# Prachet-Dev-Singh/DenseCLIP_Vit_multimodal

Hardware: AMD Instinct MI355X
Metric: images/sec (fwd+bwd) ViT-B/16 DenseCLIP @1024x2048 (higher is better)
Workload: dtype bf16

## Files before the change

denseclip_vit_multimodal_amd/csrc/attention_bwd1.hip:

```cpp
#include "dkdv_frag.h"

namespace {

constexpr int B1_NW = 4, B1_KB = 64 * B1_NW;
typedef Dkv2Ctx<bf16, B1_NW> B1Ring;
constexpr int B1_RING = 4 * B1Ring::SLOT;
constexpr int B1_W0 = B1_RING;
constexpr int B1_SMEM = B1_W0 + B1_KB * 4;
constexpr int B1_IMG = B1_KB * 128;
static_assert(B1_SMEM + 2 * B1_IMG <= 160 * 1024, "LDS");

__device__ __forceinline__ int lane_now() {
    int l;
    asm volatile("v_mbcnt_lo_u32_b32 %0, -1, 0\n\tv_mbcnt_hi_u32_b32 %0, -1, %0" : "=v"(l));
    return l;
}

template <typename F>
__device__ __forceinline__ F to_agpr(F v) {
    F r;
    asm volatile("" : "=a"(r) : "0"(v));
    return r;
}

// ... 92 lines not shown
    seeds(S0, P0, nb, nsub, h);
    fence();
}

template <typename T>
__device__ __forceinline__ void dq_tile(f32x16& acc, const char* kimg, const char* dsimg, int qb, int db) {
    typedef typename Mfma<T>::frag frag;
    const int lane = threadIdx.x & 63;
    const DsTrBase dsb = ds_tr_base(qb, lane);
    frag a[2], b[2];
    a[0] = tr_frag<T>(kimg, 0, 0, db, lane);
    b[0] = trds_frag<T>(dsimg, dsb, 0, 0);
    acc = zero16();
#pragma unroll
    for (int ks = 0; ks < 16; ++ks) {
        if (ks + 1 < 16) {
            a[(ks + 1) & 1] = tr_frag<T>(kimg, (ks + 1) >> 1, (ks + 1) & 1, db, lane);
            b[(ks + 1) & 1] = trds_frag<T>(dsimg, dsb, (ks + 1) >> 1, (ks + 1) & 1);
        }
        acc = Mfma<T>::mma(a[ks & 1], b[ks & 1], acc);
    }
}

template <typename T>
__device__ __forceinline__ void store_dq_half(rsrc_t rp, uint32_t rs, uint32_t row0, int db, const f32x16& acc,
                                              float scale) {
    typedef T t2 __attribute__((ext_vector_type(2)));
    unsigned w[4][2];
#pragma unroll
    for (int g = 0; g < 4; ++g)
#pragma unroll
        for (int j = 0; j < 2; ++j) {
            const float a0 = acc[4 * g + 2 * j], a1 = acc[4 * g + 2 * j + 1];
            const t2 p = std::is_same<T, bf16>::value ? t2{(T)a0, (T)a1} : t2{(T)(a0 * scale), (T)(a1 * scale)};
            w[g][j] = __builtin_bit_cast(unsigned, p);
        }
    const int lane = lane_now();
    const uint32_t vo = (uint32_t)(lane & 31) * rs + (uint32_t)(16 * (lane >> 5) + 64 * db);
    const uint32_t so = row0 * rs;
    typedef unsigned u32x4 __attribute__((ext_vector_type(4)));
#pragma unroll
    for (int G = 0; G < 4; G += 2) {
#pragma unroll
        for (int j = 0; j < 2; ++j) {
            const auto r = __builtin_amdgcn_permlane32_swap(w[G][j], w[G + 1][j], false, false);
            w[G][j] = r[0];
            w[G + 1][j] = r[1];
        }
        const u32x4 v = {w[G][0], w[G][1], w[G + 1][0], w[G + 1][1]};
        __builtin_amdgcn_raw_buffer_store_b128(v, rp, vo + 16 * G, so, 0);
    }
}

struct B1Out {
    rsrc_t part;
    uint32_t rs;
    int qb, db;
    float sc;
};

template <typename T, int Q>
__device__ __forceinline__ void step1(Dkv2Ctx<T, 4>& c, K6<T>& k, int t, typename Mfma<T>::frag (&qa)[4],
                                      typename Mfma<T>::frag (&ga)[4], f32x16& S0, f32x16& P0, f32x16& dq,
                                      const B1Out& out, char* kimg, char* dsimg) {
    typedef Dkv2Ctx<T, 4> X;
    wait_vmcnt<X::PIECES + 1>();
    __builtin_amdgcn_s_barrier();
    asm volatile("" ::: "memory");
    if (t > 0)
        store_dq_half<T>(out.part, out.rs, (uint32_t)(64 * (t - 1) + 1 + out.qb * 32), out.db, dq, out.sc);
    dkv2_issue<T, 4>(c, t + 3 < c.nt ? t + 3 : c.nt - 1, (Q + 3) & 3);
    const char* cur = c.smem + Q * X::SLOT;
    const char* nxt = c.smem + ((Q + 1) & 3) * X::SLOT;
    sub1<T, 0>(k, c.h, c.l32, c.lane, cur, cur, 1, qa, ga, S0, P0, dsimg, c.wave);
    sub1<T, 1>(k, c.h, c.l32, c.lane, cur, nxt, 0, qa, ga, S0, P0, dsimg, c.wave);
    asm volatile("s_waitcnt lgkmcnt(0)" ::: "memory");
    __builtin_amdgcn_s_barrier();
    asm volatile("" ::: "memory");
    fence();
    dq_tile<T>(dq, kimg, dsimg, out.qb, out.db);
    fence();
}

template <typename T>
__global__ __launch_bounds__(256, 1) void attn_bwd1_kernel(const T* __restrict__ qkv, const T* __restrict__ dout,
                                                           const float* __restrict__ lse,
                                                           const float* __restrict__ delta,
                                                           const float* __restrict__ nlse,
                                                           const float* __restrict__ ndelta, T* __restrict__ dqkv,
                                                           T* __restrict__ dqpart, int N, int H, float dk_scale,
                                                           float scale, float* __restrict__ r0q) {
    constexpr int NW = B1_NW, KB = B1_KB;
    typedef Dkv2Ctx<T, NW> X;
    typedef typename Mfma<T>::frag frag;
    static_assert(X::SLOT == B1Ring::SLOT, "ring geometry");
    __shared__ __attribute__((aligned(128))) char smem[B1_SMEM];
    __shared__ __attribute__((aligned(128))) char kimg[B1_IMG];
    __shared__ __attribute__((aligned(128))) char dsimg[B1_IMG];
    X c;
    K6<T> k;
    c.smem = smem;
    c.lane = threadIdx.x & 63;
    c.wave = __builtin_amdgcn_readfirstlane(threadIdx.x >> 6);
    c.h = c.lane >> 5;
    c.l32 = c.lane & 31;
    const int nkb = (N - 1 + KB - 1) / KB;
    const int tile = xcd_remap(blockIdx.x, gridDim.x);
    const int kblk = tile % nkb, bh = tile / nkb, b = bh / H, hd = bh % H;
    const int C = H * HD;
    const int64_t ld = 3 * (int64_t)C;
    const T* Bb = qkv + (int64_t)b * N * ld;
// ... 312 lines not shown
        fence();
        asm volatile("" : "+a"(k.vf[1][s]));
        P1 = Mfma<T>::mma(ga[s], k.vf[1][s], P1);
        fin_chunk<T>(S0, P0, k0, 2 * s + 1);
        fence();
    }
    dq_mma2<T, 8 * SUB + 2, false>(dq, kt, dbf);
    fence();
    dq_load2<T, 8 * SUB + 4>(dbf, dsprev, dqo);
#pragma unroll
    for (int s = 0; s < 2; ++s) {
        mfma_acc<T, false>(k.dv[0][0], gt[s][0], as_frag<T>(k0.p[s]));
        fin_chunk<T>(S1, P1, k1, 4 * s);
        fence();
        mfma_acc<T, false>(k.dv[0][1], gt[s][1], as_frag<T>(k0.p[s]));
        fin_chunk<T>(S1, P1, k1, 4 * s + 1);
        fence();
        mfma_acc<T, false>(k.dk[0][0], qt[s][0], as_frag<T>(k0.d[s]));
        fin_chunk<T>(S1, P1, k1, 4 * s + 2);
        fence();
        mfma_acc<T, false>(k.dk[0][1], qt[s][1], as_frag<T>(k0.d[s]));
        fin_chunk<T>(S1, P1, k1, 4 * s + 3);
        fence();
    }
    load_qg_x<T>(qa, ga, nb, nsub, l32, h);
    dq_mma2<T, 8 * SUB + 4, false>(dq, kt, dbf);
    fence();
    dq_load2<T, 8 * SUB + 6>(dbf, dsprev, dqo);
    const uint32_t dsw = ds_put_base(wave, lane);
    ds_put<SUB, 0>(dscur, dsw, k0.d);
#pragma unroll
    for (int s = 0; s < 2; ++s) {
        mfma_acc<T, true>(k.dv[1][0], gt[s][0], as_frag<T>(k1.p[s]));
        mfma_acc<T, false>(k.dv[1][1], gt[s][1], as_frag<T>(k1.p[s]));
        mfma_acc<T, false>(k.dk[1][0], qt[s][0], as_frag<T>(k1.d[s]));
        mfma_acc<T, false>(k.dk[1][1], qt[s][1], as_frag<T>(k1.d[s]));
    }
    ds_put<SUB, 1>(dscur, dsw, k1.d);
    seeds(S0, P0, nb, nsub, h);
    dq_mma2<T, 8 * SUB + 6, false>(dq, kt, dbf);
    fence();
}

template <typename T, int Q, int DB>
__device__ __forceinline__ void step2(Dkv2Ctx<T, 4>& c, K6<T>& k, int t, typename Mfma<T>::frag (&qa)[4],
                                      typename Mfma<T>::frag (&ga)[4], f32x16& S0, f32x16& P0, f32x16& dq,
                                      const B1Out& out, const DqOps& dqo, const typename Mfma<T>::frag (&kt)[16],
                                      char* dsimg) {
    typedef Dkv2Ctx<T, 4> X;
    wait_vmcnt<X::PIECES + 1>();
    asm volatile("s_waitcnt lgkmcnt(0)" ::: "memory");
    __builtin_amdgcn_s_barrier();
    asm volatile("" ::: "memory");
    dkv2_issue<T, 4>(c, t + 3 < c.nt ? t + 3 : c.nt - 1, (Q + 3) & 3);
    const char* cur = c.smem + Q * X::SLOT;
    const char* nxt = c.smem + ((Q + 1) & 3) * X::SLOT;
    char* dscur = dsimg + DB * B1_IMG;
    const char* dsprev = dsimg + (DB ^ 1) * B1_IMG;
    sub2<T, 0>(k, c.h, c.l32, c.lane, c.wave, cur, cur, 1, qa, ga, S0, P0, dq, kt, dscur, dsprev, dqo, &out,
               t >= 2 ? (uint32_t)(64 * (t - 2) + 1 + out.qb * 32) : 0xFFFFFFFFu);
    sub2<T, 1>(k, c.h, c.l32, c.lane, c.wave, cur, nxt, 0, qa, ga, S0, P0, dq, kt, dscur, dsprev, dqo);
}

template <typename T>
__device__ __forceinline__ void dq_tile_kt(f32x16& acc, const typename Mfma<T>::frag (&kt)[16], const char* dsimg,
                                           const DqOps& dqo) {
    typename Mfma<T>::frag b[2];
    dq_load2<T, 0>(b, dsimg, dqo);
    dq_mma2<T, 0, true>(acc, kt, b);
#pragma unroll
    for (int ks = 2; ks < 16; ks += 2) {
        switch (ks) {
            case 2: dq_load2<T, 2>(b, dsimg, dqo); dq_mma2<T, 2, false>(acc, kt, b); break;
            case 4: dq_load2<T, 4>(b, dsimg, dqo); dq_mma2<T, 4, false>(acc, kt, b); break;
            case 6: dq_load2<T, 6>(b, dsimg, dqo); dq_mma2<T, 6, false>(acc, kt, b); break;
            case 8: dq_load2<T, 8>(b, dsimg, dqo); dq_mma2<T, 8, false>(acc, kt, b); break;
            case 10: dq_load2<T, 10>(b, dsimg, dqo); dq_mma2<T, 10, false>(acc, kt, b); break;
            case 12: dq_load2<T, 12>(b, dsimg, dqo); dq_mma2<T, 12, false>(acc, kt, b); break;
            default: dq_load2<T, 14>(b, dsimg, dqo); dq_mma2<T, 14, false>(acc, kt, b); break;
        }
    }
}

template <typename T>
struct B1pArgs {
    const T *qkv, *dout;
    const float *lse, *delta, *nlse, *ndelta;
    T *dqkv, *dqpart;
    int N, H;
    float dk_scale, scale;
    float* r0q;
    int tiles, nbh;
    int period;
    unsigned* state;
    const float* ds0v;
};

template <typename T, bool P>
__device__ __forceinline__ int bwd1b_tile(const T* __restrict__ qkv, const T* __restrict__ dout,
                                          const float* __restrict__ lse, const float* __restrict__ delta,
                                          const float* __restrict__ nlse, const float* __restrict__ ndelta,
                                          T* __restrict__ dqkv, T* __restrict__ dqpart, int N, int H, float dk_scale,
                                          float scale, float* __restrict__ r0q, int tile, int pend, int wave,
                                          __attribute__((address_space(4))) const B1pArgs<T>* ka) {
    constexpr int NW = B1_NW, KB = B1_KB;
    typedef Dkv2Ctx<T, NW> X;
    typedef typename Mfma<T>::frag frag;
    static_assert(X::SLOT == B1Ring::SLOT, "ring geometry");
    __shared__ __attribute__((aligned(128))) char smem[B2_SMEM];
    __shared__ __attribute__((aligned(128))) char dsimg[2 * B1_IMG];
    char* kimg = dsimg + B1_IMG;
    X c;
    K6<T> k;
    c.smem = smem;
    c.lane = P ? lane_now() : (int)(threadIdx.x & 63);
    c.wave = P ? wave : __builtin_amdgcn_readfirstlane(threadIdx.x >> 6);
    if constexpr (P) asm volatile("" : "+s"(N), "+s"(H), "+s"(c.wave));
    c.h = c.lane >> 5;
    c.l32 = c.lane & 31;
    const int nkb = (N - 1 + KB - 1) / KB;
    const int kblk = tile % nkb, bh = tile / nkb, b = bh / H, hd = bh % H;
    const int C = H * HD;
    const int64_t ld = 3 * (int64_t)C;
    const T* Bb = qkv + (int64_t)b * N * ld;
    const T* dOb = dout + (int64_t)b * N * C;
    c.ldq = (uint32_t)(ld * sizeof(T));
    c.ldg = (uint32_t)(C * sizeof(T));
    c.nt = (N - 1 + 63) / 64;
    c.rem = N - 1 - 64 * (c.nt - 1);
    B1Out out;
    out.rs = (uint32_t)nkb * 128;
    out.part = make_rsrc((const char*)dqpart + ((size_t)bh * (size_t)(1 + 64 * c.nt) * nkb + kblk) * 128,
                         (uint32_t)(1 + 64 * c.nt) * out.rs);
    out.qb = c.wave >> 1;
    out.db = c.wave & 1;
    out.sc = scale / DsScale<T>::v;
    DqOps dqo;
    dqo.db = out.db;
    dqo.dsb = ds_tr_base(out.qb, c.lane);
    int key[2];
    bool kok[2];
#pragma unroll
    for (int kb = 0; kb < 2; ++kb) {
        key[kb] = 1 + kblk * KB + c.wave * 64 + kb * 32 + c.l32;
        kok[kb] = key[kb] < N;
        const int kc = kok[kb] ? key[kb] : N - 1;
#pragma unroll
        for (int s = 0; s < 4; ++s) {
            k.kf[kb][s] = *(const frag*)(Bb + (int64_t)kc * ld + C + hd * HD + (2 * s + c.h) * 8);
            k.vf[kb][s] = *(const frag*)(Bb + (int64_t)kc * ld + 2 * C + hd * HD + (2 * s + c.h) * 8);
        }
    }
    frag q0[4], g0[4];
#pragma unroll
    for (int s = 0; s < 4; ++s) {
        q0[s] = *(const frag*)(Bb + hd * HD + (2 * s + c.h) * 8);
        g0[s] = *(const frag*)(dOb + hd * HD + (2 * s + c.h) * 8);
    }
    typedef T t4 __attribute__((ext_vector_type(4)));
    t4 q0d[2][4], g0d[2][4];
#pragma unroll
    for (int db = 0; db < 2; ++db)
#pragma unroll
        for (int g = 0; g < 4; ++g) {
            q0d[db][g] = *(const t4*)(Bb + hd * HD + db * 32 + 8 * g + 4 * c.h);
            g0d[db][g] = *(const t4*)(dOb + hd * HD + db * 32 + 8 * g + 4 * c.h);
        }
    const float L0 = lse[(int64_t)bh * N], d0 = delta[(int64_t)bh * N];

    c.rs = make_rsrc(Bb, (uint32_t)N * c.ldq);
    c.rg = make_rsrc(dOb, (uint32_t)N * c.ldg);
    c.rl = make_rsrc(nlse + (int64_t)bh * N, (uint32_t)N * 4);
    c.rd = make_rsrc(ndelta + (int64_t)bh * N, (uint32_t)N * 4);
    const bool q_wave = c.wave * X::PIECES < 8;
    c.rmine = q_wave ? c.rs : c.rg;
    c.ldmine = q_wave ? c.ldq : c.ldg;
#pragma unroll
    for (int i = 0; i < X::PIECES; ++i) {
        const int piece = c.wave * X::PIECES + i;
        const int r = (piece & 7) * 8 + (c.lane >> 3);
        const uint32_t chunk = (uint32_t)(((c.lane & 7) ^ xsw(r)) * 16);
        c.voff[i] = piece < 8 ? (uint32_t)r * c.ldq + chunk + (uint32_t)(hd * HD * sizeof(T))
                              : (uint32_t)r * c.ldg + chunk + (uint32_t)(hd * HD * sizeof(T));
    }
    dkv2_issue<T, NW>(c, 0, 0);
    dkv2_issue<T, NW>(c, c.nt > 1 ? 1 : 0, 1);
    dkv2_issue<T, NW>(c, c.nt > 2 ? 2 : c.nt - 1, 2);

#pragma unroll
    for (int kb = 0; kb < 2; ++kb) {
        const int row = c.wave * 64 + kb * 32 + c.l32;
#pragma unroll
        for (int s = 0; s < 4; ++s) {
            frag v = k.kf[kb][s];
            if (!kok[kb])
#pragma unroll
                for (int j = 0; j < 8; ++j) v[j] = (T)0.f;
            *(frag*)(kimg + row * 128 + (((2 * s + c.h) ^ xsw(row)) << 4)) = v;
        }
    }
#pragma unroll
    for (int kb = 0; kb < 2; ++kb) {
        float spart = 0.f, ppart = 0.f;
#pragma unroll
        for (int s = 0; s < 4; ++s)
#pragma unroll
            for (int j = 0; j < 8; ++j) {
                spart += (float)q0[s][j] * (float)k.kf[kb][s][j];
                ppart += (float)g0[s][j] * (float)k.vf[kb][s][j];
            }
        const float p0 = __builtin_amdgcn_exp2f(xhalf_sum(spart) - L0);
        const float ds0 = p0 * (xhalf_sum(ppart) - d0) * DsScale<T>::v;
        ((float*)(smem + B2_RING))[c.wave * 64 + kb * 32 + c.l32] = kok[kb] ? ds0 : 0.f;
#pragma unroll
        for (int db = 0; db < 2; ++db)
#pragma unroll
            for (int g = 0; g < 4; ++g)
#pragma unroll
                for (int e = 0; e < 4; ++e) {
                    k.dv[kb][db][4 * g + e] = p0 * (float)g0d[db][g][e];
                    k.dk[kb][db][4 * g + e] = ds0 * (float)q0d[db][g][e];
                }
#pragma unroll
        for (int s = 0; s < 4; ++s) frag_ds_scale<T>(k.vf[kb][s]);
    }

    wait_vmcnt<2 * (X::PIECES + 1)>();
    asm volatile("s_waitcnt lgkmcnt(0)" ::: "memory");
    __builtin_amdgcn_s_barrier();
    asm volatile("" ::: "memory");
    frag qa[4], ga[4], kt[16];
    f32x16 S0, P0, dq;
#pragma unroll
    for (int ks = 0; ks < 16; ++ks) kt[ks] = to_agpr(tr_frag<T>(kimg, ks >> 1, ks & 1, dqo.db, c.lane));
    load_qg<T>(qa, ga, smem, 0, c.l32, c.h);
    seeds(S0, P0, smem, 0, c.h);
    int t = 0;
    for (; t + 4 <= c.nt; t += 4) {
        step2<T, 0, 0>(c, k, t, qa, ga, S0, P0, dq, out, dqo, kt, dsimg);
        step2<T, 1, 1>(c, k, t + 1, qa, ga, S0, P0, dq, out, dqo, kt, dsimg);
        step2<T, 2, 0>(c, k, t + 2, qa, ga, S0, P0, dq, out, dqo, kt, dsimg);
        step2<T, 3, 1>(c, k, t + 3, qa, ga, S0, P0, dq, out, dqo, kt, dsimg);
    }
    if (t < c.nt) step2<T, 0, 0>(c, k, t++, qa, ga, S0, P0, dq, out, dqo, kt, dsimg);
    if (t < c.nt) step2<T, 1, 1>(c, k, t++, qa, ga, S0, P0, dq, out, dqo, kt, dsimg);
    if (t < c.nt) step2<T, 2, 0>(c, k, t++, qa, ga, S0, P0, dq, out, dqo, kt, dsimg);
    wait_vmcnt<0>();
    asm volatile("s_waitcnt lgkmcnt(0)" ::: "memory");
    __builtin_amdgcn_s_barrier();
    asm volatile("" ::: "memory");
    if (c.nt >= 2) {
        dq_settle(dq);
        store_dq_half<T>(out.part, out.rs, (uint32_t)(64 * (c.nt - 2) + 1 + out.qb * 32), out.db, dq, out.sc);
    }
    dq_tile_kt<T>(dq, kt, dsimg + ((c.nt - 1) & 1) * B1_IMG, dqo);
    dq_settle(dq);
    store_dq_half<T>(out.part, out.rs, (uint32_t)(64 * (c.nt - 1) + 1 + out.qb * 32), out.db, dq, out.sc);
    wait_vmcnt<0>();
    unsigned duty = 0;
    if (r0q != nullptr) {
        __syncthreads();
        const int lane = P ? lane_now() : (int)__lane_id();
        float* part = (float*)(smem + NW * 64 * 128);
        gu32* state = nullptr;
        if constexpr (P) {
            asm volatile("" : "+s"(ka));
            state = (gu32*)ka->state;
            if (c.wave == NW - 1 && lane == 0) {
                __builtin_amdgcn_fence(__ATOMIC_RELEASE, "agent");
                asm volatile("s_waitcnt vmcnt(0)" ::: "memory");
                __hip_atomic_fetch_add(state + bh, 1u, __ATOMIC_RELAXED, __HIP_MEMORY_SCOPE_AGENT);
                unsigned ready = 0;
                for (int j = 0; j < pend; ++j) {
                    const int u = tile - (j + 1) * (int)gridDim.x;
                    if (u >= 0 && __hip_atomic_load(state + u / nkb, __ATOMIC_RELAXED, __HIP_MEMORY_SCOPE_AGENT) ==
                                      (unsigned)nkb)
                        ready |= 1u << j;
                }
                ((unsigned*)part)[NW * 64] = ready;
            }
        }
        char* img = smem + c.wave * 64 * 128;
        r0_put<T>(img, k.kf[0], lane & 31, lane >> 5);
        r0_put<T>(img, k.kf[1], 32 + (lane & 31), lane >> 5);
        const float aq = r0_colsum<T, 64>(img, (const float*)(smem + B2_RING) + c.wave * 64, lane);
        part[c.wave * 64 + lane] = aq;
        __syncthreads();
        if constexpr (P) {
            duty = __builtin_amdgcn_readfirstlane(((const unsigned*)part)[NW * 64]);
            if (duty && c.wave == NW - 1 && lane == 0) {
                __builtin_amdgcn_fence(__ATOMIC_ACQUIRE, "agent");
                asm volatile("s_waitcnt vmcnt(0)" ::: "memory");
            }
        }
        if (c.wave == 0) {
            float sum = 0.f;
#pragma unroll
            for (int v = 0; v < NW; ++v) sum += part[v * 64 + lane];
            r0q[((int64_t)bh * nkb + kblk) * 64 + lane] = sum;
        }
    }
    asm volatile("s_nop 7\n\ts_nop 7\n\ts_nop 3"
                 : "+a"(k.dk[0][0]), "+a"(k.dk[0][1]), "+a"(k.dk[1][0]), "+a"(k.dk[1][1]), "+a"(k.dv[0][0]),
                   "+a"(k.dv[0][1]), "+a"(k.dv[1][0]), "+a"(k.dv[1][1]));
#pragma unroll
    for (int kb = 0; kb < 2; ++kb) {
        if (kok[kb]) {
            T* rk = dqkv + ((int64_t)b * N + key[kb]) * ld + C + hd * HD;
            store_row_t21<T>(rk, k.dk[kb], dk_scale / DsScale<T>::v, c.h);
            store_row_t21<T>(rk + C, k.dv[kb], 1.0f, c.h);
        }
    }
    if constexpr (P) {
        if (duty) {
            __syncthreads();
            asm volatile("" : "+s"(ka));
            const T* pp = ka->dqpart;
            const int nrb = (N - 1 + 31) / 32, per = (nrb + nkb - 1) / nkb;
            const int tid = c.wave * 64 + lane_now();
            for (int j = 0; j < pend; ++j) {
                if (!(duty >> j & 1)) continue;
                const int u = tile - j * (int)gridDim.x, pbh = (u - (int)gridDim.x) / nkb, share = u % nkb;
                const int rb1 = min((share + 1) * per, nrb);
                for (int rb = share * per; rb < rb1; rb += DUTY_R) {
                    const int nr = min(DUTY_R, rb1 - rb);
                    dq_reduce_rows<T, DUTY_R>(pp, ka->ds0v, ka->qkv, ka->dqkv, N, H, nkb, pbh, rb, nr,
                                              ka->scale / DsScale<T>::v, tid);
                    if (tid < nr)
                        __hip_atomic_store((gu32*)ka->state + bwd1b_reduced_at(ka->nbh, pbh, nrb, rb + tid), 1u,
                                           __ATOMIC_RELAXED, __HIP_MEMORY_SCOPE_AGENT);
                }
            }
        }
        __syncthreads();
    }
    return bh;
}

template <typename T>
__global__ __launch_bounds__(256, 1) void attn_bwd1b_kernel(const T* __restrict__ qkv, const T* __restrict__ dout,
                                                            const float* __restrict__ lse,
                                                            const float* __restrict__ delta,
                                                            const float* __restrict__ nlse,
                                                            const float* __restrict__ ndelta, T* __restrict__ dqkv,
                                                            T* __restrict__ dqpart, int N, int H, float dk_scale,
                                                            float scale, float* __restrict__ r0q) {
    bwd1b_tile<T, false>(qkv, dout, lse, delta, nlse, ndelta, dqkv, dqpart, N, H, dk_scale, scale, r0q,
                         xcd_remap(blockIdx.x, gridDim.x), 0, 0, nullptr);
}

template <typename T>
__global__ __launch_bounds__(256, 1) void attn_bwd1p_kernel(const B1pArgs<T> args) {
    typedef __attribute__((address_space(4))) const B1pArgs<T> kargs_t;
    const int wave = __builtin_amdgcn_readfirstlane(threadIdx.x >> 6);
    const int period = args.period;
    int owed = 0, round = blockIdx.x / 8;
    for (int tile = xcd_remap(blockIdx.x, gridDim.x); tile < args.tiles; tile += gridDim.x, ++round) {
        kargs_t* ka = (kargs_t*)__builtin_amdgcn_kernarg_segment_ptr();
        asm volatile("" : "+s"(ka));
        ++owed;
        const bool now = period > 0 && (round % period == period - 1 || tile + (int)gridDim.x >= ka->tiles);
        bwd1b_tile<T, true>(ka->qkv, ka->dout, ka->lse, ka->delta, ka->nlse, ka->ndelta, ka->dqkv, ka->dqpart, ka->N,
                            ka->H, ka->dk_scale, ka->scale, ka->r0q, tile, now ? owed : 0, wave, ka);
        if (now || period <= 0) owed = 0;
    }
}

template <typename T>
__global__ __launch_bounds__(256) void attn_bwd1_prep_kernel(const T* __restrict__ qkv, const T* __restrict__ o,
                                                             const T* __restrict__ dout, const float* __restrict__ lse,
                                                             float* __restrict__ delta, float* __restrict__ nstat,
                                                             float* __restrict__ ds0v, float* __restrict__ r0kv, int N,
                                                             int H, int nqp, int head_minor) {
    typedef typename Mfma<T>::frag frag;
    constexpr int QB = 128;
    __shared__ __attribute__((aligned(16))) char smem[4 * 32 * 128 + 2 * QB * 4 + 4 * 128 * 4];
    const int lane = threadIdx.x & 63, wave = threadIdx.x >> 6, h = lane >> 5, l32 = lane & 31;
    int blk, bh;
    if (head_minor) {
        const int hm = blockIdx.x % H, r = blockIdx.x / H;
        blk = r % nqp;
        bh = (r / nqp) * H + hm;
    } else {
        blk = blockIdx.x % nqp;
        bh = blockIdx.x / nqp;
    }
    const int b = bh / H, hd = bh % H;
    const int C = H * HD;
    const int64_t ld = 3 * (int64_t)C;
    const T* Bb = qkv + (int64_t)b * N * ld;
    const T* dOb = dout + (int64_t)b * N * C + hd * HD;
    const int q = 1 + blk * QB + wave * 32 + l32;
    const bool qok = q < N;
    const int qc = qok ? q : N - 1;
    frag qf[4], gf[4], of[4], k0[4], v0[4];
    const T* Orow = o + ((int64_t)b * N + qc) * C + hd * HD;
#pragma unroll
    for (int s = 0; s < 4; ++s) {
        k0[s] = *(const frag*)(Bb + C + hd * HD + (2 * s + h) * 8);
        v0[s] = *(const frag*)(Bb + 2 * C + hd * HD + (2 * s + h) * 8);
        qf[s] = *(const frag*)(Bb + (int64_t)qc * ld + hd * HD + (2 * s + h) * 8);
        gf[s] = *(const frag*)(dOb + (int64_t)qc * C + (2 * s + h) * 8);
        of[s] = *(const frag*)(Orow + (2 * s + h) * 8);
    }
    const float L = lse[(int64_t)bh * N + qc];
    float dpart = 0.f, spart = 0.f, ppart = 0.f;
#pragma unroll
    for (int s = 0; s < 4; ++s)
#pragma unroll
        for (int j = 0; j < 8; ++j) {
            dpart += (float)of[s][j] * (float)gf[s][j];
            spart += (float)qf[s][j] * (float)k0[s][j];
            ppart += (float)gf[s][j] * (float)v0[s][j];
        }
    const float dl = xhalf_sum(dpart);
    const float p0 = __builtin_amdgcn_exp2f(xhalf_sum(spart) - L);
// ... 42 lines not shown
    if (state != nullptr && __hip_atomic_load((const gu32*)state + bwd1b_reduced_at(gridDim.x / nrb, bh, nrb, rb),
                                              __ATOMIC_RELAXED, __HIP_MEMORY_SCOPE_AGENT) != 0)
        return;
    dq_reduce_rows<T, 1>(dqpart, ds0v, qkv, dqkv, N, H, nkb, bh, rb, 1, sc, threadIdx.x);
}

constexpr int RQ_Q = 8;
constexpr int RQ_MAX_NKB = 56;
template <typename T>
__global__ __launch_bounds__(256) void attn_bwd1_dq_reduce_lds(const T* __restrict__ dqpart,
                                                               const float* __restrict__ ds0v,
                                                               const T* __restrict__ qkv, T* __restrict__ dqkv,
                                                               int N, int H, int nkb, int nrb, float sc,
                                                               const unsigned* state) {
    typedef T t2 __attribute__((ext_vector_type(2)));
    typedef unsigned u32x4 __attribute__((ext_vector_type(4)));
    extern __shared__ __attribute__((aligned(16))) char rq_lds[];
    const int rb = blockIdx.x % nrb, bh = blockIdx.x / nrb, b = bh / H, hd = bh % H;
    if (state != nullptr &&
        __hip_atomic_load((const gu32*)state + bwd1b_reduced_at(gridDim.x / nrb, bh, (N - 1 + 31) / 32, rb / (32 / RQ_Q)),
                          __ATOMIC_RELAXED, __HIP_MEMORY_SCOPE_AGENT) != 0)
        return;
    const int q0 = 1 + rb * RQ_Q;
    const int C = H * HD;
    const int64_t ld = 3 * (int64_t)C;
    const int64_t Np = 1 + 64 * (int64_t)((N - 1 + 63) / 64);
    const int run = nkb * 128, stride = run + 128;
    const char* src = (const char*)(dqpart + ((int64_t)bh * Np + q0) * nkb * 64);
    const int chunks = RQ_Q * nkb * 8;
    for (int c = threadIdx.x; c < chunks; c += 256) {
        const int qi = c / (nkb * 8), w = c - qi * (nkb * 8);
        const u32x4 v = __builtin_nontemporal_load((const u32x4*)(src + (int64_t)c * 16));
        *(u32x4*)(rq_lds + qi * stride + w * 16) = v;
    }
    __syncthreads();
    const int qi = threadIdx.x >> 5, cp = threadIdx.x & 31;
    const int q = q0 + qi;
    if (q >= N) return;
    const t2 kv = *(const t2*)(qkv + (int64_t)b * N * ld + C + hd * HD + 2 * cp);
    constexpr bool unscaled = std::is_same<T, bf16>::value;
    const float w = ds0v[(int64_t)bh * N + q] * (unscaled ? 1.0f : sc);
    float a0 = w * (float)kv[0], a1 = w * (float)kv[1];
    const char* row = rq_lds + qi * stride + cp * 4;
#pragma unroll 8
    for (int j = 0; j < nkb; ++j) {
        const t2 v = *(const t2*)(row + j * 128);
        a0 += (float)v[0];
        a1 += (float)v[1];
    }
    const t2 r = {(T)(unscaled ? a0 * sc : a0), (T)(unscaled ? a1 * sc : a1)};
    *(t2*)(dqkv + ((int64_t)b * N + q) * ld + hd * HD + 2 * cp) = r;
}

int bwd1_cu_count() {
    int dev = 0, c = 0;
    if (hipGetDevice(&dev) != hipSuccess ||
        hipDeviceGetAttribute(&c, hipDeviceAttributeMultiprocessorCount, dev) != hipSuccess || c <= 0)
        c = 256;
    return c;
}

template <typename T>
void bwd1_launch(const void* qkv, const void* o, const void* dout, const float* lse, float* delta, float* nstat,
                 float* ds0v, float* r0kv, int nqp, float* r0q, void* dqpart, void* dqkv, int B, int N, int H,
                 float scale, unsigned* state, hipStream_t st) {
    const int nkb = (N - 1 + B1_KB - 1) / B1_KB, tiles = B * H * nkb;
    attn_bwd1_prep_kernel<T><<<B * H * nqp, 256, 0, st>>>((const T*)qkv, (const T*)o, (const T*)dout, lse, delta, nstat,
                                                          ds0v, r0kv, N, H, nqp,
                                                          dclip_option(DCLIP_OPT_ATTN_PREP_ORDER) == 1);
    const int blk = dclip_option(DCLIP_OPT_ATTN_BWD_BLOCK), cap = dclip_option(DCLIP_OPT_ATTN_BWD_WGS);
    const int G = cap > 0 ? cap : bwd1_cu_count();
    const bool persistent = blk == 0 && state != nullptr && r0q != nullptr && tiles > G;
    if (!persistent) state = nullptr;
    if (persistent) {
        (void)hipMemsetAsync(state, 0, (size_t)attn_bwd1_state_bytes(B, N, H), st);
        const B1pArgs<T> args = {(const T*)qkv, (const T*)dout, lse,   delta,  nstat, nstat + (int64_t)B * H * N,
                                 (T*)dqkv,      (T*)dqpart,     N,     H,      1.0f / LOG2E, scale,
                                 r0q,           tiles,          B * H, DUTY_PERIOD, state, ds0v};
        attn_bwd1p_kernel<T><<<G, 256, 0, st>>>(args);
    } else if (blk != 9)
        attn_bwd1b_kernel<T><<<B * H * nkb, 256, 0, st>>>((const T*)qkv, (const T*)dout, lse, delta, nstat,
                                                          nstat + (int64_t)B * H * N, (T*)dqkv, (T*)dqpart, N, H,
                                                          1.0f / LOG2E, scale, r0q);
    else
        attn_bwd1_kernel<T><<<B * H * nkb, 256, 0, st>>>((const T*)qkv, (const T*)dout, lse, delta, nstat,
                                                         nstat + (int64_t)B * H * N, (T*)dqkv, (T*)dqpart, N, H,
                                                         1.0f / LOG2E, scale, r0q);
    if (dclip_option(DCLIP_OPT_ATTN_DQ_REDUCE) == 1 && nkb <= RQ_MAX_NKB) {
        const int nrb = (N - 1 + RQ_Q - 1) / RQ_Q;
        attn_bwd1_dq_reduce_lds<T><<<B * H * nrb, 256, RQ_Q * (nkb * 128 + 128), st>>>(
            (const T*)dqpart, ds0v, (const T*)qkv, (T*)dqkv, N, H, nkb, nrb, scale / DsScale<T>::v, state);
        return;
    }
    const int nrb = (N - 1 + 31) / 32;
    attn_bwd1_dq_reduce<T><<<B * H * nrb, 256, 0, st>>>((const T*)dqpart, ds0v, (const T*)qkv, (T*)dqkv, N, H, nkb, nrb,
                                                        scale / DsScale<T>::v, state);
}

}

int attn_bwd1_prep_blocks(int N) { return (N - 1 + 127) / 128; }

int64_t attn_bwd1_part_bytes(int B, int N, int H) {
    const int64_t nkb = (N - 1 + B1_KB - 1) / B1_KB, np = 1 + 64 * (int64_t)((N - 1 + 63) / 64);
    return (int64_t)B * H * nkb * np * 128;
}

int64_t attn_bwd1_state_bytes(int B, int N, int H) {
    const int64_t words = (int64_t)B * H * (1 + (N - 1 + 31) / 32);
    return (words * 4 + 255) / 256 * 256;
}

void attn_bwd1_launch(int dt, const void* qkv, const void* o, const void* dout, const float* lse, float* delta,
                      float* nstat, float* ds0v, float* r0kv, float* r0q, void* dqpart, void* dqkv, int B, int N,
                      int H, float scale, hipStream_t st, void* state) {
    const int nqp = attn_bwd1_prep_blocks(N);
    if (dt == DCLIP_BF16)
        bwd1_launch<bf16>(qkv, o, dout, lse, delta, nstat, ds0v, r0kv, nqp, r0q, dqpart, dqkv, B, N, H, scale,
                          (unsigned*)state, st);
    else
        bwd1_launch<f16>(qkv, o, dout, lse, delta, nstat, ds0v, r0kv, nqp, r0q, dqpart, dqkv, B, N, H, scale,
                         (unsigned*)state, st);
}
```

Measured before the change: 64.88.

## Prefetch next persistent tile's K/V/CLS rows into LDS across the tile seam

In the persistent attention backward kernel, the next tile's K/V rows, the CLS q/dout rows and its first three ring stages are issued as async buffer-to-LDS loads while the current tile finishes its dq tail, r0 fold and dK/dV stores. At the start of the next tile the fragments are read from LDS instead of global memory. The goal is to hide global-load latency at the boundary between tiles. The r0 fold is moved earlier into a dedicated LDS region, __syncthreads calls are replaced with raw barriers, and hipMemsetAsync is replaced with a small zeroing kernel. It also adds optional timestamp diagnostics. This costs extra LDS and adds staging-buffer aliasing hazards.

```diff
diff --git a/denseclip_vit_multimodal_amd/csrc/attention_bwd1.hip b/denseclip_vit_multimodal_amd/csrc/attention_bwd1.hip
--- a/denseclip_vit_multimodal_amd/csrc/attention_bwd1.hip
+++ b/denseclip_vit_multimodal_amd/csrc/attention_bwd1.hip
@@ -168,11 +168,43 @@
     }
 }
 
+#ifndef DCLIP_BWD1_SEAM_PREFETCH
+#define DCLIP_BWD1_SEAM_PREFETCH 1
+#endif
+enum {
+    B1_PT_RT0 = 0,
+    B1_PT_TOP = 1,
+    B1_PT_LOOP = 2,
+    B1_PT_LEFT = 3,
+    B1_PT_DQ = 4,
+    B1_PT_PUB = 5,
+    B1_PT_DKDV = 6,
+    B1_PT_END = 7,
+    B1_PT_RT1 = 8,
+    B1_PTS = 16
+};
+#ifdef DCLIP_BWD1_SEAM_DIAG
+constexpr int B1_DIAG_TILES = 4096;
+__device__ unsigned long long g_seam_stamps[B1_DIAG_TILES * B1_PTS];
+#define B1_STAMP_V(tile, pt, who, val)                                                              \
+    do {                                                                                            \
+        if ((who) && (tile) >= 0 && (tile) < B1_DIAG_TILES) g_seam_stamps[(tile) * B1_PTS + (pt)] = (val); \
+    } while (0)
+#define B1_STAMP(tile, pt, who) B1_STAMP_V(tile, pt, who, __builtin_amdgcn_s_memtime())
+#define B1_STAMP_RT(tile, pt, who) B1_STAMP_V(tile, pt, who, __builtin_amdgcn_s_memrealtime())
+#else
+#define B1_STAMP(tile, pt, who) do { } while (0)
+#define B1_STAMP_RT(tile, pt, who) do { } while (0)
+#endif
+
 struct B1Out {
     rsrc_t part;
     uint32_t rs;
     int qb, db;
     float sc;
+#ifdef DCLIP_BWD1_SEAM_DIAG
+    int diag_tile;
+#endif
 };
 
 template <typename T, int Q>
@@ -591,6 +623,9 @@
     asm volatile("s_waitcnt lgkmcnt(0)" ::: "memory");
     __builtin_amdgcn_s_barrier();
     asm volatile("" ::: "memory");
+#ifdef DCLIP_BWD1_SEAM_DIAG
+    if constexpr (Q == 0) B1_STAMP(out.diag_tile, B1_PT_LOOP, t == 0 && c.wave == 0 && lane_now() == 0);
+#endif
     dkv2_issue<T, 4>(c, t + 3 < c.nt ? t + 3 : c.nt - 1, (Q + 3) & 3);
     const char* cur = c.smem + Q * X::SLOT;
     const char* nxt = c.smem + ((Q + 1) & 3) * X::SLOT;
@@ -635,30 +670,30 @@
     const float* ds0v;
 };
 
-template <typename T, bool P>
-__device__ __forceinline__ int bwd1b_tile(const T* __restrict__ qkv, const T* __restrict__ dout,
-                                          const float* __restrict__ lse, const float* __restrict__ delta,
-                                          const float* __restrict__ nlse, const float* __restrict__ ndelta,
-                                          T* __restrict__ dqkv, T* __restrict__ dqpart, int N, int H, float dk_scale,
-                                          float scale, float* __restrict__ r0q, int tile, int pend, int wave,
-                                          __attribute__((address_space(4))) const B1pArgs<T>* ka) {
-    constexpr int NW = B1_NW, KB = B1_KB;
-    typedef Dkv2Ctx<T, NW> X;
-    typedef typename Mfma<T>::frag frag;
-    static_assert(X::SLOT == B1Ring::SLOT, "ring geometry");
-    __shared__ __attribute__((aligned(128))) char smem[B2_SMEM];
-    __shared__ __attribute__((aligned(128))) char dsimg[2 * B1_IMG];
-    char* kimg = dsimg + B1_IMG;
-    X c;
-    K6<T> k;
-    c.smem = smem;
-    c.lane = P ? lane_now() : (int)(threadIdx.x & 63);
-    c.wave = P ? wave : __builtin_amdgcn_readfirstlane(threadIdx.x >> 6);
-    if constexpr (P) asm volatile("" : "+s"(N), "+s"(H), "+s"(c.wave));
+constexpr int B1_CLS = B2_RING;
+constexpr int B1_FOLD_W0 = 0, B1_FOLD_PART = B1_KB * 4, B1_FOLD_READY = B1_FOLD_PART + B1_NW * 64 * 4;
+constexpr int B1_FOLD = B1_FOLD_READY + 128;
+constexpr int B1_VST = (B1_NW - 1) * 64 * 128;
+static_assert(B2_SMEM + 2 * B1_IMG + B1_FOLD + B1_VST <= 160 * 1024, "LDS");
+static_assert(64 * 128 <= B1Ring::SLOT, "wave 3's V stage in ring slot 3");
+
+template <typename T>
+struct B1Pre {
+    typename Mfma<T>::frag kf[2][4], vf[2][4];
+    typename Mfma<T>::frag q0[4], g0[4];
+    typedef T t4 __attribute__((ext_vector_type(4)));
+    t4 q0d[2][4], g0d[2][4];
+};
+
+template <typename T>
+__device__ __forceinline__ void b1_ring_ctx(Dkv2Ctx<T, B1_NW>& c, const T* __restrict__ qkv,
+                                            const T* __restrict__ dout, const float* __restrict__ nlse,
+                                            const float* __restrict__ ndelta, int N, int H, int tile) {
+    typedef Dkv2Ctx<T, B1_NW> X;
     c.h = c.lane >> 5;
     c.l32 = c.lane & 31;
-    const int nkb = (N - 1 + KB - 1) / KB;
-    const int kblk = tile % nkb, bh = tile / nkb, b = bh / H, hd = bh % H;
+    const int nkb = (N - 1 + B1_KB - 1) / B1_KB;
+    const int bh = tile / nkb, b = bh / H, hd = bh % H;
     const int C = H * HD;
     const int64_t ld = 3 * (int64_t)C;
     const T* Bb = qkv + (int64_t)b * N * ld;
@@ -667,6 +702,157 @@
     c.ldg = (uint32_t)(C * sizeof(T));
     c.nt = (N - 1 + 63) / 64;
     c.rem = N - 1 - 64 * (c.nt - 1);
+    c.rs = make_rsrc(Bb, (uint32_t)N * c.ldq);
+    c.rg = make_rsrc(dOb, (uint32_t)N * c.ldg);
+    c.rl = make_rsrc(nlse + (int64_t)bh * N, (uint32_t)N * 4);
+    c.rd = make_rsrc(ndelta + (int64_t)bh * N, (uint32_t)N * 4);
+    const bool q_wave = c.wave * X::PIECES < 8;
+    c.rmine = q_wave ? c.rs : c.rg;
+    c.ldmine = q_wave ? c.ldq : c.ldg;
+#pragma unroll
+    for (int i = 0; i < X::PIECES; ++i) {
+        const int piece = c.wave * X::PIECES + i;
+        const int r = (piece & 7) * 8 + (c.lane >> 3);
+        const uint32_t chunk = (uint32_t)(((c.lane & 7) ^ xsw(r)) * 16);
+        c.voff[i] = piece < 8 ? (uint32_t)r * c.ldq + chunk + (uint32_t)(hd * HD * sizeof(T))
+                              : (uint32_t)r * c.ldg + chunk + (uint32_t)(hd * HD * sizeof(T));
+    }
+}
+
+template <typename T>
+__device__ __forceinline__ void b1_tile_loads(B1Pre<T>& p, Dkv2Ctx<T, B1_NW>& c, const T* __restrict__ qkv,
+                                              const T* __restrict__ dout, int N, int H, int tile) {
+    typedef typename Mfma<T>::frag frag;
+    const int nkb = (N - 1 + B1_KB - 1) / B1_KB;
+    const int kblk = tile % nkb, bh = tile / nkb, b = bh / H, hd = bh % H;
+    const int C = H * HD;
+    const int64_t ld = 3 * (int64_t)C;
+    const T* Bb = qkv + (int64_t)b * N * ld;
+    const T* dOb = dout + (int64_t)b * N * C;
+#pragma unroll
+    for (int kb = 0; kb < 2; ++kb) {
+        const int key = 1 + kblk * B1_KB + c.wave * 64 + kb * 32 + c.l32;
+        const int kc = key < N ? key : N - 1;
+#pragma unroll
+        for (int s = 0; s < 4; ++s) {
+            p.kf[kb][s] = *(const frag*)(Bb + (int64_t)kc * ld + C + hd * HD + (2 * s + c.h) * 8);
+            p.vf[kb][s] = *(const frag*)(Bb + (int64_t)kc * ld + 2 * C + hd * HD + (2 * s + c.h) * 8);
+        }
+    }
+#pragma unroll
+    for (int s = 0; s < 4; ++s) {
+        p.q0[s] = *(const frag*)(Bb + hd * HD + (2 * s + c.h) * 8);
+        p.g0[s] = *(const frag*)(dOb + hd * HD + (2 * s + c.h) * 8);
+    }
+    typedef typename B1Pre<T>::t4 t4;
+#pragma unroll
+    for (int db = 0; db < 2; ++db)
+#pragma unroll
+        for (int g = 0; g < 4; ++g) {
+            p.q0d[db][g] = *(const t4*)(Bb + hd * HD + db * 32 + 8 * g + 4 * c.h);
+            p.g0d[db][g] = *(const t4*)(dOb + hd * HD + db * 32 + 8 * g + 4 * c.h);
+        }
+    dkv2_issue<T, B1_NW>(c, 0, 0);
+    dkv2_issue<T, B1_NW>(c, c.nt > 1 ? 1 : 0, 1);
+    dkv2_issue<T, B1_NW>(c, c.nt > 2 ? 2 : c.nt - 1, 2);
+}
+
+template <typename T, bool V>
+__device__ __forceinline__ void b1_stage_rows(const Dkv2Ctx<T, B1_NW>& c, char* dst, int N, int H, int tile) {
+#if defined(__HIP_DEVICE_COMPILE__)
+    const int nkb = (N - 1 + B1_KB - 1) / B1_KB;
+    const int kblk = tile % nkb, hd = (tile / nkb) % H;
+    const uint32_t col = (uint32_t)(((V ? 2 : 1) * H * HD + hd * HD) * sizeof(T));
+#pragma unroll
+    for (int i = 0; i < 8; ++i) {
+        const int r = 8 * i + (c.lane >> 3);
+        const int key = 1 + kblk * B1_KB + c.wave * 64 + r;
+        const uint32_t kc = (uint32_t)(key < N ? key : N - 1);
+        __builtin_amdgcn_raw_ptr_buffer_load_lds(c.rs, LDS_PTR(dst + i * 1024), 16,
+                                                 kc * c.ldq + col + (uint32_t)(((c.lane & 7) ^ xsw(r)) * 16), 0, 0, 0);
+    }
+#endif
+}
+
+template <typename T>
+__device__ __forceinline__ void b1_stage_cls(const Dkv2Ctx<T, B1_NW>& c, char* dst, int N, int H, int tile) {
+#if defined(__HIP_DEVICE_COMPILE__)
+    const int nkb = (N - 1 + B1_KB - 1) / B1_KB;
+    const int hd = (tile / nkb) % H;
+    const uint32_t off = (uint32_t)(hd * HD * sizeof(T)) + (uint32_t)((c.lane & 7) * 16);
+    if (c.lane < 8) __builtin_amdgcn_raw_ptr_buffer_load_lds(c.rs, LDS_PTR(dst), 16, off, 0, 0, 0);
+    if (c.lane >= 8 && c.lane < 16) __builtin_amdgcn_raw_ptr_buffer_load_lds(c.rg, LDS_PTR(dst), 16, off, 0, 0, 0);
+#endif
+}
+
+template <typename T>
+__device__ __forceinline__ void b1_stage_reads(B1Pre<T>& p, const Dkv2Ctx<T, B1_NW>& c, const char* kst,
+                                               const char* vst, const char* cls) {
+    typedef typename Mfma<T>::frag frag;
+#pragma unroll
+    for (int kb = 0; kb < 2; ++kb)
+#pragma unroll
+        for (int s = 0; s < 4; ++s) {
+            p.kf[kb][s] = row_frag<T>(kst, kb * 32 + c.l32, 2 * s + c.h);
+            p.vf[kb][s] = row_frag<T>(vst, kb * 32 + c.l32, 2 * s + c.h);
+        }
+#pragma unroll
+    for (int s = 0; s < 4; ++s) {
+        p.q0[s] = *(const frag*)(cls + (2 * s + c.h) * 16);
+        p.g0[s] = *(const frag*)(cls + 128 + (2 * s + c.h) * 16);
+    }
+    typedef typename B1Pre<T>::t4 t4;
+#pragma unroll
+    for (int db = 0; db < 2; ++db)
+#pragma unroll
+        for (int g = 0; g < 4; ++g) {
+            p.q0d[db][g] = *(const t4*)(cls + (db * 32 + 8 * g + 4 * c.h) * 2);
+            p.g0d[db][g] = *(const t4*)(cls + 128 + (db * 32 + 8 * g + 4 * c.h) * 2);
+        }
+}
+
+__device__ __forceinline__ char* b1_kstage(char* dsimg, int nt, int wave) {
+    return dsimg + (nt & 1) * B1_IMG + wave * 64 * 128;
+}
+__device__ __forceinline__ char* b1_vstage(char* vst, char* smem, int wave) {
+    return wave < B1_NW - 1 ? vst + wave * 64 * 128 : smem + 3 * B1Ring::SLOT;
+}
+
+template <typename T, bool P>
+__device__ __forceinline__ int bwd1b_tile(const T* __restrict__ qkv, const T* __restrict__ dout,
+                                          const float* __restrict__ lse, const float* __restrict__ delta,
+                                          const float* __restrict__ nlse, const float* __restrict__ ndelta,
+                                          T* __restrict__ dqkv, T* __restrict__ dqpart, int N, int H, float dk_scale,
+                                          float scale, float* __restrict__ r0q, int tile, int pend, int wave,
+                                          __attribute__((address_space(4))) const B1pArgs<T>* ka, char* smem,
+                                          char* dsimg, char* fold, char* vst, int next_tile) {
+    constexpr int NW = B1_NW, KB = B1_KB;
+    typedef Dkv2Ctx<T, NW> X;
+    typedef typename Mfma<T>::frag frag;
+    static_assert(X::SLOT == B1Ring::SLOT, "ring geometry");
+    char* kimg = dsimg + B1_IMG;
+    X c;
+    K6<T> k;
+    c.smem = smem;
+    c.lane = P ? lane_now() : (int)(threadIdx.x & 63);
+    c.wave = P ? wave : __builtin_amdgcn_readfirstlane(threadIdx.x >> 6);
+    if constexpr (P) asm volatile("" : "+s"(N), "+s"(H), "+s"(c.wave));
+    const int nkb = (N - 1 + KB - 1) / KB;
+    const int kblk = tile % nkb, bh = tile / nkb, b = bh / H, hd = bh % H;
+    const int C = H * HD;
+    const int64_t ld = 3 * (int64_t)C;
+    b1_ring_ctx<T>(c, qkv, dout, nlse, ndelta, N, H, tile);
+    B1_STAMP_RT(tile, B1_PT_RT0, P && c.wave == 0 && c.lane == 0);
+    B1_STAMP(tile, B1_PT_TOP, P && c.wave == 0 && c.lane == 0);
+    constexpr bool STAGED = P && DCLIP_BWD1_SEAM_PREFETCH != 0;
+    B1Pre<T> pre;
+    if constexpr (STAGED) {
+        wait_vmcnt<0>();
+        b1_stage_reads<T>(pre, c, b1_kstage(dsimg, c.nt, c.wave), b1_vstage(vst, smem, c.wave),
+                          smem + B1_CLS + c.wave * 256);
+    } else {
+        b1_tile_loads<T>(pre, c, qkv, dout, N, H, tile);
+    }
     B1Out out;
     out.rs = (uint32_t)nkb * 128;
     out.part = make_rsrc((const char*)dqpart + ((size_t)bh * (size_t)(1 + 64 * c.nt) * nkb + kblk) * 128,
@@ -674,6 +860,9 @@
     out.qb = c.wave >> 1;
     out.db = c.wave & 1;
     out.sc = scale / DsScale<T>::v;
+#ifdef DCLIP_BWD1_SEAM_DIAG
+    out.diag_tile = P ? tile : -1;
+#endif
     DqOps dqo;
     dqo.db = out.db;
     dqo.dsb = ds_tr_base(out.qb, c.lane);
@@ -683,48 +872,28 @@
     for (int kb = 0; kb < 2; ++kb) {
         key[kb] = 1 + kblk * KB + c.wave * 64 + kb * 32 + c.l32;
         kok[kb] = key[kb] < N;
-        const int kc = kok[kb] ? key[kb] : N - 1;
 #pragma unroll
         for (int s = 0; s < 4; ++s) {
-            k.kf[kb][s] = *(const frag*)(Bb + (int64_t)kc * ld + C + hd * HD + (2 * s + c.h) * 8);
-            k.vf[kb][s] = *(const frag*)(Bb + (int64_t)kc * ld + 2 * C + hd * HD + (2 * s + c.h) * 8);
+            k.kf[kb][s] = pre.kf[kb][s];
+            k.vf[kb][s] = pre.vf[kb][s];
         }
     }
     frag q0[4], g0[4];
 #pragma unroll
     for (int s = 0; s < 4; ++s) {
-        q0[s] = *(const frag*)(Bb + hd * HD + (2 * s + c.h) * 8);
-        g0[s] = *(const frag*)(dOb + hd * HD + (2 * s + c.h) * 8);
-    }
-    typedef T t4 __attribute__((ext_vector_type(4)));
+        q0[s] = pre.q0[s];
+        g0[s] = pre.g0[s];
+    }
+    typedef typename B1Pre<T>::t4 t4;
     t4 q0d[2][4], g0d[2][4];
 #pragma unroll
     for (int db = 0; db < 2; ++db)
 #pragma unroll
         for (int g = 0; g < 4; ++g) {
-            q0d[db][g] = *(const t4*)(Bb + hd * HD + db * 32 + 8 * g + 4 * c.h);
-            g0d[db][g] = *(const t4*)(dOb + hd * HD + db * 32 + 8 * g + 4 * c.h);
+            q0d[db][g] = pre.q0d[db][g];
+            g0d[db][g] = pre.g0d[db][g];
         }
     const float L0 = lse[(int64_t)bh * N], d0 = delta[(int64_t)bh * N];
-
-    c.rs = make_rsrc(Bb, (uint32_t)N * c.ldq);
-    c.rg = make_rsrc(dOb, (uint32_t)N * c.ldg);
-    c.rl = make_rsrc(nlse + (int64_t)bh * N, (uint32_t)N * 4);
-    c.rd = make_rsrc(ndelta + (int64_t)bh * N, (uint32_t)N * 4);
-    const bool q_wave = c.wave * X::PIECES < 8;
-    c.rmine = q_wave ? c.rs : c.rg;
-    c.ldmine = q_wave ? c.ldq : c.ldg;
-#pragma unroll
-    for (int i = 0; i < X::PIECES; ++i) {
-        const int piece = c.wave * X::PIECES + i;
-        const int r = (piece & 7) * 8 + (c.lane >> 3);
-        const uint32_t chunk = (uint32_t)(((c.lane & 7) ^ xsw(r)) * 16);
-        c.voff[i] = piece < 8 ? (uint32_t)r * c.ldq + chunk + (uint32_t)(hd * HD * sizeof(T))
-                              : (uint32_t)r * c.ldg + chunk + (uint32_t)(hd * HD * sizeof(T));
-    }
-    dkv2_issue<T, NW>(c, 0, 0);
-    dkv2_issue<T, NW>(c, c.nt > 1 ? 1 : 0, 1);
-    dkv2_issue<T, NW>(c, c.nt > 2 ? 2 : c.nt - 1, 2);
 
 #pragma unroll
     for (int kb = 0; kb < 2; ++kb) {
@@ -750,7 +919,7 @@
             }
         const float p0 = __builtin_amdgcn_exp2f(xhalf_sum(spart) - L0);
         const float ds0 = p0 * (xhalf_sum(ppart) - d0) * DsScale<T>::v;
-        ((float*)(smem + B2_RING))[c.wave * 64 + kb * 32 + c.l32] = kok[kb] ? ds0 : 0.f;
+        ((float*)(fold + B1_FOLD_W0))[c.wave * 64 + kb * 32 + c.l32] = kok[kb] ? ds0 : 0.f;
 #pragma unroll
         for (int db = 0; db < 2; ++db)
 #pragma unroll
@@ -788,6 +957,7 @@
     asm volatile("s_waitcnt lgkmcnt(0)" ::: "memory");
     __builtin_amdgcn_s_barrier();
     asm volatile("" ::: "memory");
+    B1_STAMP(tile, B1_PT_LEFT, P && c.wave == 0 && lane_now() == 0);
     if (c.nt >= 2) {
         dq_settle(dq);
         store_dq_half<T>(out.part, out.rs, (uint32_t)(64 * (c.nt - 2) + 1 + out.qb * 32), out.db, dq, out.sc);
@@ -795,16 +965,43 @@
     dq_tile_kt<T>(dq, kt, dsimg + ((c.nt - 1) & 1) * B1_IMG, dqo);
     dq_settle(dq);
     store_dq_half<T>(out.part, out.rs, (uint32_t)(64 * (c.nt - 1) + 1 + out.qb * 32), out.db, dq, out.sc);
+    const bool do_fold = r0q != nullptr;
+    const int lane = P ? lane_now() : (int)__lane_id();
+    float* part = (float*)(fold + B1_FOLD_PART);
+    if (do_fold) {
+        char* img = b1_kstage(dsimg, c.nt, c.wave);
+        r0_put<T>(img, k.kf[0], lane & 31, lane >> 5);
+        r0_put<T>(img, k.kf[1], 32 + (lane & 31), lane >> 5);
+        const float aq = r0_colsum<T, 64>(img, (const float*)(fold + B1_FOLD_W0) + c.wave * 64, lane);
+        part[c.wave * 64 + lane] = aq;
+    }
     wait_vmcnt<0>();
+    asm volatile("s_waitcnt lgkmcnt(0)" ::: "memory");
+    B1_STAMP(tile, B1_PT_DQ, P && c.wave == 0 && lane_now() == 0);
+    auto stage_next = [&]() {
+        asm volatile("" : "+s"(ka));
+        X cn;
+        cn.smem = smem;
+        cn.lane = lane_now();
+        cn.wave = c.wave;
+        b1_ring_ctx<T>(cn, ka->qkv, ka->dout, ka->nlse, ka->ndelta, N, H, next_tile);
+        b1_stage_rows<T, false>(cn, b1_kstage(dsimg, c.nt, c.wave), N, H, next_tile);
+        b1_stage_rows<T, true>(cn, b1_vstage(vst, smem, c.wave), N, H, next_tile);
+        b1_stage_cls<T>(cn, smem + B1_CLS + c.wave * 256, N, H, next_tile);
+        dkv2_issue<T, NW>(cn, 0, 0);
+        dkv2_issue<T, NW>(cn, cn.nt > 1 ? 1 : 0, 1);
+        dkv2_issue<T, NW>(cn, cn.nt > 2 ? 2 : cn.nt - 1, 2);
+    };
+    if constexpr (STAGED) {
+        if (next_tile >= 0 && c.wave != NW - 1) stage_next();
+    }
     unsigned duty = 0;
-    if (r0q != nullptr) {
-        __syncthreads();
-        const int lane = P ? lane_now() : (int)__lane_id();
-        float* part = (float*)(smem + NW * 64 * 128);
-        gu32* state = nullptr;
+    if (do_fold) {
+        __builtin_amdgcn_s_barrier();
+        asm volatile("" ::: "memory");
         if constexpr (P) {
             asm volatile("" : "+s"(ka));
-            state = (gu32*)ka->state;
+            gu32* state = (gu32*)ka->state;
             if (c.wave == NW - 1 && lane == 0) {
                 __builtin_amdgcn_fence(__ATOMIC_RELEASE, "agent");
                 asm volatile("s_waitcnt vmcnt(0)" ::: "memory");
@@ -816,27 +1013,31 @@
                                       (unsigned)nkb)
                         ready |= 1u << j;
                 }
-                ((unsigned*)part)[NW * 64] = ready;
+                *(unsigned*)(fold + B1_FOLD_READY) = ready;
+#ifdef DCLIP_BWD1_SEAM_DIAG
+                asm volatile("s_waitcnt vmcnt(0)" ::: "memory");
+                B1_STAMP(tile, B1_PT_PUB, true);
+#endif
             }
-        }
-        char* img = smem + c.wave * 64 * 128;
-        r0_put<T>(img, k.kf[0], lane & 31, lane >> 5);
-        r0_put<T>(img, k.kf[1], 32 + (lane & 31), lane >> 5);
-        const float aq = r0_colsum<T, 64>(img, (const float*)(smem + B2_RING) + c.wave * 64, lane);
-        part[c.wave * 64 + lane] = aq;
-        __syncthreads();
+            if constexpr (STAGED) {
+                if (next_tile >= 0 && c.wave == NW - 1) stage_next();
+            }
+        }
+        if (c.wave == 0) {
+            float sum = 0.f;
+#pragma unroll
+            for (int v = 0; v < NW; ++v) sum += part[v * 64 + lane];
+            r0q[((int64_t)bh * nkb + kblk) * 64 + lane] = sum;
+        }
         if constexpr (P) {
-            duty = __builtin_amdgcn_readfirstlane(((const unsigned*)part)[NW * 64]);
+            asm volatile("s_waitcnt lgkmcnt(0)" ::: "memory");
+            __builtin_amdgcn_s_barrier();
+            asm volatile("" ::: "memory");
+            duty = __builtin_amdgcn_readfirstlane(*(const unsigned*)(fold + B1_FOLD_READY));
             if (duty && c.wave == NW - 1 && lane == 0) {
                 __builtin_amdgcn_fence(__ATOMIC_ACQUIRE, "agent");
                 asm volatile("s_waitcnt vmcnt(0)" ::: "memory");
             }
-        }
-        if (c.wave == 0) {
-            float sum = 0.f;
-#pragma unroll
-            for (int v = 0; v < NW; ++v) sum += part[v * 64 + lane];
-            r0q[((int64_t)bh * nkb + kblk) * 64 + lane] = sum;
         }
     }
     asm volatile("s_nop 7\n\ts_nop 7\n\ts_nop 3"
@@ -850,6 +1051,7 @@
             store_row_t21<T>(rk + C, k.dv[kb], 1.0f, c.h);
         }
     }
+    B1_STAMP(tile, B1_PT_DKDV, P && c.wave == 0 && lane_now() == 0);
     if constexpr (P) {
         if (duty) {
             __syncthreads();
@@ -871,7 +1073,11 @@
                 }
             }
         }
-        __syncthreads();
+        asm volatile("s_waitcnt lgkmcnt(0)" ::: "memory");
+        __builtin_amdgcn_s_barrier();
+        asm volatile("" ::: "memory");
+        B1_STAMP(tile, B1_PT_END, c.wave == 0 && lane_now() == 0);
+        B1_STAMP_RT(tile, B1_PT_RT1, c.wave == 0 && lane_now() == 0);
     }
     return bh;
 }
@@ -884,8 +1090,11 @@
                                                             const float* __restrict__ ndelta, T* __restrict__ dqkv,
                                                             T* __restrict__ dqpart, int N, int H, float dk_scale,
                                                             float scale, float* __restrict__ r0q) {
+    __shared__ __attribute__((aligned(128))) char smem[B2_SMEM];
+    __shared__ __attribute__((aligned(128))) char dsimg[2 * B1_IMG];
+    __shared__ __attribute__((aligned(128))) char fold[B1_FOLD];
     bwd1b_tile<T, false>(qkv, dout, lse, delta, nlse, ndelta, dqkv, dqpart, N, H, dk_scale, scale, r0q,
-                         xcd_remap(blockIdx.x, gridDim.x), 0, 0, nullptr);
+                         xcd_remap(blockIdx.x, gridDim.x), 0, 0, nullptr, smem, dsimg, fold, nullptr, -1);
 }
 
 template <typename T>
@@ -894,13 +1103,35 @@
     const int wave = __builtin_amdgcn_readfirstlane(threadIdx.x >> 6);
     const int period = args.period;
     int owed = 0, round = blockIdx.x / 8;
-    for (int tile = xcd_remap(blockIdx.x, gridDim.x); tile < args.tiles; tile += gridDim.x, ++round) {
+    __shared__ __attribute__((aligned(128))) char smem[B2_SMEM];
+    __shared__ __attribute__((aligned(128))) char dsimg[2 * B1_IMG];
+    __shared__ __attribute__((aligned(128))) char fold[B1_FOLD];
+    __shared__ __attribute__((aligned(128))) char vst[B1_VST];
+    int tile = xcd_remap(blockIdx.x, gridDim.x);
+    if constexpr (DCLIP_BWD1_SEAM_PREFETCH != 0) {
+        if (tile < args.tiles) {
+            Dkv2Ctx<T, B1_NW> c0;
+            c0.smem = smem;
+            c0.lane = lane_now();
+            c0.wave = wave;
+            b1_ring_ctx<T>(c0, args.qkv, args.dout, args.nlse, args.ndelta, args.N, args.H, tile);
+            b1_stage_rows<T, false>(c0, b1_kstage(dsimg, c0.nt, wave), args.N, args.H, tile);
+            b1_stage_rows<T, true>(c0, b1_vstage(vst, smem, wave), args.N, args.H, tile);
+            b1_stage_cls<T>(c0, smem + B1_CLS + wave * 256, args.N, args.H, tile);
+            dkv2_issue<T, B1_NW>(c0, 0, 0);
+            dkv2_issue<T, B1_NW>(c0, c0.nt > 1 ? 1 : 0, 1);
+            dkv2_issue<T, B1_NW>(c0, c0.nt > 2 ? 2 : c0.nt - 1, 2);
+        }
+    }
+    for (; tile < args.tiles; tile += gridDim.x, ++round) {
         kargs_t* ka = (kargs_t*)__builtin_amdgcn_kernarg_segment_ptr();
         asm volatile("" : "+s"(ka));
         ++owed;
-        const bool now = period > 0 && (round % period == period - 1 || tile + (int)gridDim.x >= ka->tiles);
+        const bool last = tile + (int)gridDim.x >= ka->tiles;
+        const bool now = period > 0 && (round % period == period - 1 || last);
         bwd1b_tile<T, true>(ka->qkv, ka->dout, ka->lse, ka->delta, ka->nlse, ka->ndelta, ka->dqkv, ka->dqpart, ka->N,
-                            ka->H, ka->dk_scale, ka->scale, ka->r0q, tile, now ? owed : 0, wave, ka);
+                            ka->H, ka->dk_scale, ka->scale, ka->r0q, tile, now ? owed : 0, wave, ka, smem, dsimg,
+                            fold, vst, last ? -1 : tile + (int)gridDim.x);
         if (now || period <= 0) owed = 0;
     }
 }
@@ -1049,6 +1280,11 @@
     *(t2*)(dqkv + ((int64_t)b * N + q) * ld + hd * HD + 2 * cp) = r;
 }
 
+__global__ __launch_bounds__(256) void attn_bwd1_zero_state(unsigned* __restrict__ state, int words) {
+    const int i = blockIdx.x * 256 + threadIdx.x;
+    if (i < words) state[i] = 0u;
+}
+
 int bwd1_cu_count() {
     int dev = 0, c = 0;
     if (hipGetDevice(&dev) != hipSuccess ||
@@ -1070,7 +1306,8 @@
     const bool persistent = blk == 0 && state != nullptr && r0q != nullptr && tiles > G;
     if (!persistent) state = nullptr;
     if (persistent) {
-        (void)hipMemsetAsync(state, 0, (size_t)attn_bwd1_state_bytes(B, N, H), st);
+        const int words = (int)(attn_bwd1_state_bytes(B, N, H) / 4);
+        attn_bwd1_zero_state<<<(words + 255) / 256, 256, 0, st>>>(state, words);
         const B1pArgs<T> args = {(const T*)qkv, (const T*)dout, lse,   delta,  nstat, nstat + (int64_t)B * H * N,
                                  (T*)dqkv,      (T*)dqpart,     N,     H,      1.0f / LOG2E, scale,
                                  r0q,           tiles,          B * H, DUTY_PERIOD, state, ds0v};
@@ -1119,3 +1356,16 @@
         bwd1_launch<f16>(qkv, o, dout, lse, delta, nstat, ds0v, r0kv, nqp, r0q, dqpart, dqkv, B, N, H, scale,
                          (unsigned*)state, st);
 }
+
+#ifdef DCLIP_BWD1_SEAM_DIAG
+extern "C" int dclip_diag_seam_stamps(void* dst, int64_t bytes) {
+    const size_t all = sizeof(unsigned long long) * B1_DIAG_TILES * B1_PTS;
+    const size_t n = bytes < (int64_t)all ? (size_t)bytes : all;
+    if (hipDeviceSynchronize() != hipSuccess) return -1;
+    if (hipMemcpyFromSymbol(dst, HIP_SYMBOL(g_seam_stamps), n) != hipSuccess) return -1;
+    void* p = nullptr;
+    if (hipGetSymbolAddress(&p, HIP_SYMBOL(g_seam_stamps)) != hipSuccess || hipMemset(p, 0, all) != hipSuccess)
+        return -1;
+    return B1_PTS;
+}
+#endif
```

Result: no change. 65.31 (median of 6 runs) (+0.7%).
